# vpulab/GNN-CCA

Hardware: AMD Instinct MI355X
Metric: processed edges/sec (L=4 MPN steps), 256-node dense graph (higher is better)
Workload: dtype f32; 1 GPU; 1 x dense256 per GPU per step (N=256, E=65280), feat 2048, L=4, 3 cls steps, fp32, fp32 state, eval; mode=eager: MOTMPNet.forward, one call per step (auto: fastest one-at-a-time form), frames_in_flight=1, edge_state=fp32, edge_state_storage=f32, encoder_products=6, encoder_unsplit=False, outputs_finite=True, launcher=single process, ranks_seen=1

## Files before the change

gnn-cca_amd/csrc/internal.h:

```cpp
#pragma once
#include <stddef.h>
#include <stdint.h>

#include "gnncca_mpn.h"

namespace gnncca {

extern thread_local int g_last_hip_error;

const char* diag_env(const char* name);
int diag_env_int(const char* name, int fallback, int lo, int hi);

constexpr uint32_t kBlobMagic = 0x4D504E36u;
constexpr int kH = 32;
constexpr int kEF = 6;
constexpr int kProjOut = 48;
constexpr int kPdStride = 8;
constexpr int kPsQStride = 40;
constexpr int kMaxCls = 8;
constexpr int kMaxEdgeIn = 16;

enum Family : uint32_t {
    kFamilyNone = 0,
    kFamilyMfma32x6 = 1,
// ... 88 lines not shown
    auto take = [&at](auto*& field, int64_t count) { field = reinterpret_cast<decltype(+field)>(at), at += sizeof(*field) * (size_t)count; };
    StagingImage s;
    take(s.xw, n), take(s.yw, n), take(s.max_dist, g), take(s.ids, n), take(s.person, n), take(s.cam, n), take(s.graph_of, n);
    take(s.graph_ptr, g + 1), take(s.src_order, n), take(s.edge_ptr, n + 1), take(s.edge_ptr_g, g + 1);
    s.bytes = at - reinterpret_cast<uintptr_t>(base);
    return s;
}
inline size_t staging_image_bytes(int64_t n, int64_t g) { return n < 0 || g < 0 ? 0 : staging_image(nullptr, n, g).bytes; }

int build_edges_zeroing(const gnncca_frames* fr, const float* reid, int32_t reid_dim, int64_t n_nodes, int64_t n_edges, int32_t mode, bool capped,
                        int32_t top_k, int32_t rank_by, int32_t max_deg, int64_t* edge_index_out, float* edge_attr_out, float* edge_labels_out,
                        int32_t* zero_ptr, int64_t zero_n, gnncca_stream_t stream);

int build_edges_radius_zeroing(const gnncca_frames* fr, const float* reid, int32_t reid_dim, int64_t n_nodes, int64_t n_edges, int32_t mode,
                               double radius, int32_t unit, int64_t* edge_index_out, float* edge_attr_out, float* edge_labels_out,
                               int32_t* zero_ptr, int64_t zero_n, gnncca_stream_t stream);

Family classify(const gnncca_mpn_dims* d);
bool blob_header(const gnncca_mpn_dims* d, BlobHeader* out);
bool dims_valid(const gnncca_mpn_dims* d);
int mlp_param_count(const gnncca_mlp& m);

struct Workspace {
    size_t flags, blockflags, seg_ptr, col32, perm, cursor, h0, act, partial, pd[2], psq[2], e, e0, rng, total;
    int ksplit;
    int64_t e_stride;
    int ell_S;
};
int ell_stride(const gnncca_mpn_dims* d, int64_t n, int64_t e);
int enc_lds_ksplit(int64_t n_nodes, int K);
Workspace carve(const gnncca_mpn_dims* d, int64_t n, int64_t e);

enum EncForm : int {
    kEncPlanGemm = 0,
    kEncSlices,
    kEncD128,
    kEncR32Bf16,
    kEncR32F16,
    kEncLdsBf16,
    kEncLdsF16,
};
enum EncPlanPlace : int {
    kPlanNone = 0,
    kPlanRides,
    kPlanBefore,
    kPlanAfter,
};
// ... 34 lines not shown
    int kslice;
    int nst;
    int vec_ok;
};
struct EncRoute {
    int n_gemm;
    EncGemmRoute gemm[GNNCCA_MAX_LAYERS];
    bool split3, fused;
    int x_nt, force_arm;
    int plan_place, plan_span, plan_wgs;
    int tail, tail_npw, tail_vec;
    size_t tail_lds;
};
EncRoute encoder_route(const EncRouteIn& in, const EncTuning& t);

enum StepFamily : int {
    kStepGeneral = 0,
    kStepFast,
    kStepPipe,
};
#ifndef GNNCCA_NPW2_CLS
#define GNNCCA_NPW2_CLS 0
#endif
constexpr bool step_variant_exists(int family, bool FIRST, bool CLS, bool MSG, bool PDL, bool EB, int NT, bool RNG, int NPW, bool CIN) {
    if (family == kStepGeneral) return true;
    if (NT < 0 || NT > 2 || (NT != 0 && PDL)) return false;
    if (family == kStepFast) return !RNG && NPW == 1 && !CIN;
    if (CIN) return !FIRST && !PDL && !EB && !RNG && (MSG ? !CLS && (NPW == 1 || NPW == 2) : CLS && NPW == 1);
    if (RNG) return NT == 0 && NPW == 1;
    if (NPW == 2) return MSG && !PDL && (!CLS || GNNCCA_NPW2_CLS);
    return NPW == 1;
}
inline bool step_pipe_fits(long long N, long long E, long long e_stride, unsigned long long ws_bytes) {
    const long long lim = 1ll << 31;
    return 6 * e_stride * 4 <= lim && E * 16 <= lim && N * 32 <= lim && ws_bytes <= (unsigned long long)lim - 4096;
}
struct StepTuning {
    int msg_f32_max_n = 512;
    int fill_waves = 4096, fill_waves_long = 16384;
    int long_chunks = 32;
    int npw_min_n = 16384;
    int npw_min_n_first = 16384;
    int pd_lds_min = 0x7FFFFFFF, pd_lds_max = 1024;
    double nt_store_bytes = 150e6;
    double nt_load_bytes = 256e6;
    int force_wps = 0;
    int force_npw = 0;
    int force_nt = -1;
};
const StepTuning& step_tuning();
struct StepRouteIn {
    const gnncca_mpn_dims* d;
    const BlobHeader* hdr;
    const Workspace* ws;
    int N, E;
    uint32_t options;
    bool dropping;
    bool traced, trace_h_steps;
    bool attr_aligned;
};
struct StepPlan {
    int launches;
    int family;
    bool RE, MX;
    int N, hin;
    int msg_f32, attr_vec, wps, npw_first, npw_later, pd_lds, e_bf16;
    int nt;
    bool ranges;
    int ell_S;
    bool defer;
    bool trace_h_steps;
    int first_cls, L, cls_layers;
};
struct StepLaunch {
    int family;
    bool RE, MX, FIRST, CLS, MSG, PDL, EB;
    int NT;
    bool RNG;
    int NPW;
    bool CIN;
    unsigned blocks;
    size_t lds;
    int first, update, store_e, npw, cls_layers, cls_no, stamp_slot;
    int slot_out, slot_in;
    int buf_in, buf_out;
};
StepPlan step_plan(const StepRouteIn& in, const StepTuning& t);
StepLaunch step_launch(const StepPlan& p, int step);

struct BwdWorkspace {
    size_t gh0_acc, ge0_acc;
    size_t deg, Q;
    size_t hmax;
    size_t dP_all;
    size_t Hb[2], Gb[2], a1, gz1;
    size_t part;
    size_t bn_sums, bn_red;
    size_t total;
};
inline BwdWorkspace carve_backward(const gnncca_mpn_dims* d, int64_t n, int64_t e) {
    BwdWorkspace w;
    size_t off = 0;
    auto take = [&](size_t bytes) { size_t o = off; off += (bytes + 255) / 256 * 256; return o; };
    const size_t N = (size_t)(n > 0 ? n : 0), E = (size_t)(e > 0 ? e : 0), F1 = (size_t)d->enc_node.layers[0].out_dim;
    const size_t L = (size_t)(d->num_enc_steps > 1 ? d->num_enc_steps : 1);
    w.gh0_acc = take(N * kH * 4), w.ge0_acc = take(E * kEF * 4), w.deg = take(N * 4), w.Q = take(N * kH * 4);
    w.hmax = take(2 * N * kH * 4), w.dP_all = take(L * N * 44 * 4);
    for (int i = 0; i < 2; ++i) w.Hb[i] = take(N * kH * 4);
// ... 48 lines not shown
```

gnn-cca_amd/csrc/mpn_forward.hip:

```cpp
#include "forward_diag.cuh"
#include "wave_reduce.cuh"
#include "plan.cuh"
#include "encoder.cuh"
#include "enc_rows32.cuh"
#include "msg_bf16.cuh"
#include "step_general.cuh"
#include "step_fast.cuh"
#include "step_pipe.cuh"
#include "enc_f16.cuh"
#include "enc_f16_slices.cuh"
#include "generic_fused.cuh"
#include "generic.cuh"
#include "with_flag.h"

using namespace gnncca;

extern "C" {

#ifdef GNNCCA_STAMPS
__attribute__((visibility("default"))) int gnncca_debug_set_stamps(void* dev_buf) {
    unsigned long long* p = static_cast<unsigned long long*>(dev_buf);
    HIP_TRY(hipMemcpyToSymbol(HIP_SYMBOL(g_stamps), &p, sizeof(p)));
    return GNNCCA_OK;
}
// ... 5 lines not shown
    if (!workspace || !flags_out) return GNNCCA_ERR_INVALID_ARG;
    hipStream_t st = static_cast<hipStream_t>(stream);
    HIP_TRY(hipMemcpyAsync(flags_out, workspace, sizeof(uint32_t), hipMemcpyDeviceToHost, st));
    HIP_TRY(hipStreamSynchronize(st));
    return GNNCCA_OK;
}

int gnncca_read_graph_flags2(const void* workspace, uint32_t flags_out[2], gnncca_stream_t stream) {
    if (!workspace || !flags_out) return GNNCCA_ERR_INVALID_ARG;
    hipStream_t st = static_cast<hipStream_t>(stream);
    HIP_TRY(hipMemcpyAsync(flags_out, workspace, 2 * sizeof(uint32_t), hipMemcpyDeviceToHost, st));
    HIP_TRY(hipStreamSynchronize(st));
    return GNNCCA_OK;
}

}

static_assert(kEncSliceMaxK == kF16SlMaxKs, "encoder_route() sizes the slices of enc_f16_slices.cuh");

struct FwdBuffers {
    char* base;
    unsigned *flags, *blockflags;
    int *seg_ptr, *col32, *perm, *cursor;
    float *h0, *act, *part, *pd[2], *psq[2], *e, *e0;
};
static FwdBuffers carve_pointers(void* workspace, const Workspace& ws) {
    char* base = static_cast<char*>(workspace);
    auto f = [base](size_t off) { return reinterpret_cast<float*>(base + off); };
    auto i = [base](size_t off) { return reinterpret_cast<int*>(base + off); };
    auto u = [base](size_t off) { return reinterpret_cast<unsigned*>(base + off); };
    return FwdBuffers{base, u(ws.flags), u(ws.blockflags), i(ws.seg_ptr), i(ws.col32), i(ws.perm), i(ws.cursor), f(ws.h0), f(ws.act), f(ws.partial),
                      {f(ws.pd[0]), f(ws.pd[1])}, {f(ws.psq[0]), f(ws.psq[1])}, f(ws.e), f(ws.e0)};
}

template <class P>
static void fill_plan_finish(P& p, const FwdBuffers& b, const int64_t* edge_index, int E) {
    p.ei = reinterpret_cast<const long long*>(edge_index);
    p.seg_ptr = b.seg_ptr, p.col32 = b.col32, p.perm = b.perm, p.cursor = b.cursor, p.flags = b.flags, p.blockflags = b.blockflags;
    p.E = E;
}

static int enc_gemm_attributes() {
    static thread_local int attr_dev = -1;
    int dev = 0;
    HIP_TRY(hipGetDevice(&dev));
    if (attr_dev == dev) return GNNCCA_OK;
    HIP_TRY(hipFuncSetAttribute(reinterpret_cast<const void*>(enc_gemm_f16_fused_kernel), hipFuncAttributeMaxDynamicSharedMemorySize, (int)kF16LdsBytes));
    HIP_TRY(hipFuncSetAttribute(reinterpret_cast<const void*>(enc_gemm_f16_split_kernel), hipFuncAttributeMaxDynamicSharedMemorySize, (int)kF16LdsBytes));
    HIP_TRY(hipFuncSetAttribute(reinterpret_cast<const void*>(enc_gemm_f16_rows32_kernel), hipFuncAttributeMaxDynamicSharedMemorySize, (int)kF16R32LdsBytes));
    const void* fns[4] = {reinterpret_cast<const void*>(enc_gemm_split_lds_kernel<false, false>),
                          reinterpret_cast<const void*>(enc_gemm_split_lds_kernel<true, false>),
                          reinterpret_cast<const void*>(enc_gemm_split_lds_kernel<false, true>),
                          reinterpret_cast<const void*>(enc_gemm_split_lds_kernel<true, true>)};
    for (const void* fn : fns) HIP_TRY(hipFuncSetAttribute(fn, hipFuncAttributeMaxDynamicSharedMemorySize, (int)kLdsGemmBytes));
    attr_dev = dev;
// ... 174 lines not shown
    sp.hin = plan.hin;
    sp.msg_f32 = plan.msg_f32;
    sp.attr_vec = plan.attr_vec;
    sp.wps = plan.wps;
    sp.npw = plan.npw_later;
    sp.pd_lds = plan.pd_lds;
    sp.e_bf16 = plan.e_bf16;
    sp.ell_S = plan.ell_S;
    sp.nt_store = plan.nt >= 1, sp.nt_load = plan.nt >= 2;
    sp.rng = plan.ranges ? reinterpret_cast<int*>(b.base + ws.rng) : nullptr;
    sp.ws_base = b.base;
    sp.ws_bytes = ws.total;
    sp.so_e = (unsigned)ws.e, sp.so_col = (unsigned)ws.col32, sp.so_perm = (unsigned)ws.perm;
    sp.drop = drop;
    return sp;
}

static hipError_t launch_step_variant(const StepLaunch& l, const StepParams& sp, hipStream_t st) {
    const dim3 grid(l.blocks), block(256);
    bool launched = false;
    auto with_nt = [&](auto&& f) {
        l.NT == 2 ? f(std::integral_constant<int, 2>{}) : l.NT == 1 ? f(std::integral_constant<int, 1>{}) : f(std::integral_constant<int, 0>{});
    };
    if (l.family == kStepGeneral) {
        with_flag(l.RE, [&](auto RE) { with_flag(l.MSG, [&](auto MSG) { with_flag(l.MX, [&](auto MX) {
            GNNCCA_LAUNCH((mpn_step_kernel<RE(), MSG(), MX()>), grid, block, l.lds, st, sp);
            launched = true;
        }); }); });
    } else {
        with_flag(l.FIRST, [&](auto FIRST) { with_flag(l.CLS, [&](auto CLS) { with_flag(l.MSG, [&](auto MSG) { with_flag(l.PDL, [&](auto PDL) {
        with_nt([&](auto NT) { with_flag(l.EB, [&](auto EB) {
            if (l.family == kStepFast) {
                if constexpr (step_variant_exists(kStepFast, FIRST(), CLS(), MSG(), PDL(), EB(), NT(), false, 1, false)) {
                    GNNCCA_LAUNCH((mpn_step_fast_kernel<FIRST(), CLS(), MSG(), PDL(), EB(), NT()>), grid, block, l.lds, st, sp);
                    launched = true;
                }
                return;
            }
            with_flag(l.RNG, [&](auto RNG) { with_flag(l.NPW == 2, [&](auto TWO) { with_flag(l.CIN, [&](auto CIN) {
                constexpr int NPW = TWO() ? 2 : 1;
                if constexpr (step_variant_exists(kStepPipe, FIRST(), CLS(), MSG(), PDL(), EB(), NT(), RNG(), NPW, CIN())) {
                    GNNCCA_LAUNCH((mpn_step_pipe_kernel<FIRST(), CLS(), MSG(), PDL(), EB(), NT(), RNG(), NPW, CIN()>), grid, block, l.lds, st, sp);
                    launched = true;
                }
            }); }); });
        }); });
        }); }); }); });
    }
    return launched ? hipGetLastError() : hipErrorInvalidValue;
}

static int forward_impl(const gnncca_mpn_dims* d, const void* packed_dev, const float* x, const int64_t* edge_index,
                        const float* edge_attr, int64_t n_nodes, int64_t n_edges, void* workspace, size_t workspace_bytes,
                        float* logits_out, const gnncca_trace* trace, gnncca_stream_t stream, Profiler* prof,
                        uint32_t options, const gnncca_dropout* dropout = nullptr) {
    if (!dims_valid(d) || n_nodes < 0 || n_edges < 0) return GNNCCA_ERR_INVALID_ARG;
    const Family fam = classify(d);
    if (fam == kFamilyNone) return GNNCCA_ERR_UNSUPPORTED;
    if (n_nodes >= (1ll << 31) - 64 || n_edges >= (1ll << 31) - 64) return GNNCCA_ERR_UNSUPPORTED;
    if (n_nodes == 0) return n_edges == 0 ? GNNCCA_OK : GNNCCA_ERR_INVALID_ARG;
    if (!packed_dev || !x || !workspace) return GNNCCA_ERR_INVALID_ARG;
// ... 35 lines not shown

    StepParams sp = step_setup(plan, d, hdr, ws, b, blob, edge_attr, N, E, drop);
    for (int i = 0; i < plan.launches; ++i) {
        const int step = plan.L == 0 ? 0 : i + 1;
        const StepLaunch l = step_launch(plan, step);
        sp.first = l.first;
        sp.update = l.update;
        sp.store_e = l.store_e;
        sp.npw = l.npw;
        sp.step_no = step;
        sp.cls_no = l.cls_no;
        sp.stamp_slot = l.stamp_slot;
        sp.cls_layers = l.cls_layers;
        sp.logits = l.slot_out >= 0 ? logits_out + (size_t)l.slot_out * E : nullptr;
        sp.logits_in = l.slot_in >= 0 ? logits_out + (size_t)l.slot_in * E : nullptr;
        sp.pd_in = l.buf_in >= 0 ? b.pd[l.buf_in] : nullptr;
        sp.so_pd = l.buf_in >= 0 ? (unsigned)ws.pd[l.buf_in] : 0u;
        sp.psq_in = l.buf_in >= 0 ? b.psq[l.buf_in] : nullptr;
        sp.pd_out = l.buf_out >= 0 ? b.pd[l.buf_out] : nullptr;
        sp.psq_out = l.buf_out >= 0 ? b.psq[l.buf_out] : nullptr;
        sp.trace_e_enc = (trace && l.first) ? trace->e_enc : nullptr;
        sp.trace_e = (trace && trace->e_steps && l.update) ? trace->e_steps + (size_t)(step - 1) * E * kEF : nullptr;
        sp.trace_h = (plan.trace_h_steps && l.update) ? trace->h_steps + (size_t)(step - 1) * N * kH : nullptr;
        HIP_TRY(launch_step_variant(l, sp, st));
        PROF_MARK(l.MSG ? GNNCCA_K_STEP : GNNCCA_K_STEP_LAST);
    }
    return GNNCCA_OK;
}

extern "C" {

int gnncca_mpn_forward(const gnncca_mpn_dims* d, const void* packed_dev, const float* x, const int64_t* edge_index,
                       const float* edge_attr, int64_t n_nodes, int64_t n_edges, void* workspace, size_t workspace_bytes,
                       float* logits_out, const gnncca_trace* trace, gnncca_stream_t stream) {
    return forward_impl(d, packed_dev, x, edge_index, edge_attr, n_nodes, n_edges, workspace, workspace_bytes, logits_out,
                        trace, stream, nullptr, 0u);
}

int gnncca_mpn_forward_ex(const gnncca_mpn_dims* d, const void* packed_dev, const float* x, const int64_t* edge_index,
                          const float* edge_attr, int64_t n_nodes, int64_t n_edges, void* workspace, size_t workspace_bytes,
                          float* logits_out, const gnncca_trace* trace, uint32_t options, gnncca_stream_t stream) {
    return forward_impl(d, packed_dev, x, edge_index, edge_attr, n_nodes, n_edges, workspace, workspace_bytes, logits_out,
                        trace, stream, nullptr, options);
}

int gnncca_mpn_forward_train(const gnncca_mpn_dims* d, const void* packed_dev, const float* x, const int64_t* edge_index,
// ... 25 lines not shown
```

gnn-cca_amd/csrc/pack.cpp:

```cpp
#include <algorithm>
#include <cmath>
#include <cstdio>
#include <cstdlib>
#include <cstring>
#include <vector>

#include "internal.h"

namespace gnncca {

thread_local int g_last_hip_error = 0;

static inline size_t align_up(size_t v, size_t a) { return (v + a - 1) / a * a; }

int mlp_param_count(const gnncca_mlp& m) {
    int n = 0;
    for (int i = 0; i < m.n_layers; ++i) n += 2 + (m.layers[i].has_bn ? 4 : 0);
    return n;
}

static bool mlp_chain_ok(const gnncca_mlp& m, int in_dim, int out_dim) {
    if (m.n_layers < 0 || m.n_layers > GNNCCA_MAX_LAYERS) return false;
    if (m.n_layers == 0) return in_dim == out_dim;
    int cur = in_dim;
// ... 596 lines not shown
    w.row32o = take(E * 4);
    w.col32o = take(E * 4);
    for (int i = 0; i < 3; ++i) w.node[i] = take(N * (size_t)nw * 4);
    w.h0 = take(N * (size_t)d->node_dim * 4);
    for (int i = 0; i < 4; ++i) w.edge[i] = take(E * (size_t)ew * 4);
    w.e0 = take(E * (size_t)d->edge_dim * 4);
    const int ks = gen_enc0_ksplit(d, n);
    w.partial = take(ks > 0 ? (size_t)ks * N * (size_t)d->enc_node.layers[0].out_dim * 4 : 0);
    {
        const size_t o1e = d->edge_mlp.n_layers > 0 ? (size_t)d->edge_mlp.layers[0].out_dim : 0;
        const size_t o1n = d->node_mlp.n_layers > 0 ? (size_t)d->node_mlp.layers[0].out_dim : 0;
        for (int i = 0; i < 2; ++i) w.tab[i] = take(N * (2 * o1e + o1n) * 4);
    }
    w.total = off;
    return w;
}

static const char* const kDiagSwitches[] = {
    "GNNCCA_DIAG", "GNNCCA_LIB", "GNNCCA_STAMPS",
    "GNNCCA_GEMM_SPLIT_MIN", "GNNCCA_GEMM_LDS_MIN", "GNNCCA_GEMM_R32F_MIN", "GNNCCA_GEMM_R32F_MAX",
    "GNNCCA_GEMM_SLICES_MIN", "GNNCCA_GEMM_SLICES_MAX", "GNNCCA_GEMM_SLICES_NKS", "GNNCCA_GEMM_SLICES_WGS",
    "GNNCCA_GEMM_BF16", "GNNCCA_GEMM_F16_ARM", "GNNCCA_GEMM_F16_XNT", "GNNCCA_TAIL_MFMA_MIN",
    "GNNCCA_WPS", "GNNCCA_NPW", "GNNCCA_NPW_MIN_N", "GNNCCA_NPW_MIN_N_FIRST",
    "GNNCCA_STEP_NT", "GNNCCA_PD_LDS_MIN", "GNNCCA_PD_LDS_MAX", "GNNCCA_NO_PAD",
    "GNNCCA_GEN_UNFUSED", "GNNCCA_COLNORM_NOLDS", "GNNCCA_POOL_CHUNK", "GNNCCA_POOL_SPIN_US"};

extern "C" char** environ;

const char* diag_env(const char* name) {
    static const bool on = [] {
        const char* v = std::getenv("GNNCCA_DIAG");
        const bool open = v != nullptr && v[0] == '1' && v[1] == '\0';
        if (open && environ) {
            for (char** e = environ; *e; ++e) {
                if (std::strncmp(*e, "GNNCCA_", 7) != 0) continue;
                const char* eq = std::strchr(*e, '=');
                const size_t len = eq ? (size_t)(eq - *e) : std::strlen(*e);
                bool known = false;
                for (const char* k : kDiagSwitches) known = known || (std::strlen(k) == len && std::strncmp(k, *e, len) == 0);
                if (!known) {
                    std::fprintf(stderr, "[gnncca] GNNCCA_DIAG=1: '%.*s' is not a switch of this build and is ignored; recognised:", (int)len, *e);
                    for (const char* k : kDiagSwitches) std::fprintf(stderr, " %s", k);
                    std::fprintf(stderr, "\n");
                }
            }
        }
        return open;
// ... 51 lines not shown
    int ks = 1;
    while (ks < 32 && row_tiles * (size_t)ks < 512 && k0 / (ks * 2) >= 64) ks *= 2;
    if (N >= 1024)
        while (ks < 8 && ((N + 127) / 128) * (size_t)ks < 512 && k0 / (ks * 2) >= 64) ks *= 2;
    if (N >= 4096) ks = std::max(ks, enc_lds_ksplit((int64_t)N, k0));
    w.ksplit = ks;
    size_t fmax = 0;
    for (int i = 0; i < d->enc_node.n_layers; ++i)
        fmax = fmax > (size_t)d->enc_node.layers[i].out_dim ? fmax : (size_t)d->enc_node.layers[i].out_dim;
    w.flags = take(256);
    w.blockflags = take((E / 256 + 2) * 4);
    w.seg_ptr = take((N + 1) * 4);
    w.col32 = take(E * 4);
    w.perm = take(E * 4);
    w.cursor = take((N + 1) * 4);
    w.h0 = take(N * kH * 4);
    w.act = take(d->enc_node.n_layers >= 3 ? 2 * N * fmax * 4 : 0);
    w.partial = take((size_t)ks * N * fmax * 4);
    for (int i = 0; i < 2; ++i) w.pd[i] = take(N * kPdStride * 4);
    for (int i = 0; i < 2; ++i) w.psq[i] = take(N * kPsQStride * 4);
    w.e = take((size_t)kEF * w.e_stride * 4);
    w.e0 = take(d->reattach_edges ? (size_t)kEF * w.e_stride * 4 : 0);
    w.rng = take(N * 16);
    w.total = off;
    return w;
}

}

extern "C" size_t gnncca_workspace_bytes(const gnncca_mpn_dims* d, int64_t n_nodes, int64_t n_edges) {
    const Family fam = classify(d);
    if (fam == kFamilyNone || n_nodes < 0 || n_edges < 0) return 0;
    if (fam == kFamilyGeneric) return carve_generic(d, n_nodes, n_edges).total;
    return carve(d, n_nodes, n_edges).total;
}
```

gnn-cca_amd/csrc/step_fast.cuh:

```cuda
#pragma once
namespace gnncca {

__device__ __forceinline__ float relu_bits(float x) { return __int_as_float(max(__float_as_int(x), 0)); }

#ifdef GNNCCA_FAST_WAVES
#define GNNCCA_FAST_ATTR __attribute__((amdgpu_waves_per_eu(GNNCCA_FAST_WAVES, GNNCCA_FAST_WAVES)))
#else
#define GNNCCA_FAST_ATTR __attribute__((amdgpu_waves_per_eu(MSG ? 4 : 1)))
#endif
template <bool FIRST, bool CLS, bool MSG, bool PD_LDS, bool EBF16, int NT>
__global__ __launch_bounds__(256) GNNCCA_FAST_ATTR void mpn_step_fast_kernel(const StepParams p) {
    extern __shared__ __attribute__((aligned(16))) float smem[];
    float* s_proj = smem;
    float* s_part = s_proj + (MSG ? kH * kProjOut : 0);
    int* s_rng = reinterpret_cast<int*>(s_part + 4 * kH);
    float* s_pd = s_part + 4 * kH + 16;
    const int tid = threadIdx.x, lane = tid & 63;
    const int wave = __builtin_amdgcn_readfirstlane(tid >> 6);
    const float* __restrict__ blob = p.blob;
    constexpr bool DERIVE = FIRST && MSG;
    typedef const float __attribute__((address_space(4))) cfloat;
    cfloat* cw = (cfloat*)(unsigned long long)(blob + p.off_fast);

    GNNCCA_STAMP(p.stamp_slot, 0);
    const int ktouch = touch_kernargs(sizeof(StepParams));
    const unsigned gflags = p.flags[0];
    const unsigned rbad = p.flags[1];
    const int wps = p.wps;
    const int wl = wps >> 1;
    const int node = (int)(blockIdx.x << (2 - wl)) + (wave >> wl);
    const int sub = wave & (wps - 1);
    const bool active = node < p.N;
    const int nclamp = active ? node : 0;
    int seg_s = p.seg_ptr[nclamp];
    int seg_t = p.seg_ptr[nclamp + 1];
    const bool use_range = !FIRST && p.rng != nullptr && rbad == 0u;
    int rs1 = 0, rl1 = 0, rd2 = 0;
    if (!FIRST && p.rng != nullptr) {
        typedef int i32x4 __attribute__((ext_vector_type(4)));
        const i32x4 r = reinterpret_cast<const i32x4*>(p.rng)[nclamp];
        rs1 = r[0], rl1 = r[1], rd2 = r[2];
    }
    asm volatile("" ::"s"(gflags), "s"(rbad), "s"(seg_s), "s"(seg_t), "s"(rs1), "s"(rl1), "s"(rd2), "s"(ktouch));
    const int nmax = p.N - 1;
    const int half = lane >> 5, ch = lane & 31;
    const float* __restrict__ psq = p.psq_in + (size_t)nclamp * kPsQStride;
    float psrc[kEF];
    float cinit = 0.f;
    float bw[3] = {0.f, 0.f, 0.f};
    f32x4 stage_proj[2];
    f32x4 stage_pd[8];
    float projb_l = 0.f;
    const int pd_n4 = p.N * (kPdStride / 4);
    auto request_node_operands = [&]() {
#pragma unroll
        for (int f = 0; f < kEF; ++f) psrc[f] = psq[f];
        if (MSG) {
            cinit = psq[8 + ch];
            projb_l = blob[p.off_projb + min(lane, kProjOut - 1)];
#pragma unroll
            for (int s = 0; s < 3; ++s) bw[s] = blob[p.off_wneb + s * 64 + lane];
            const f32x4* __restrict__ g4 = reinterpret_cast<const f32x4*>(blob + p.off_projwT);
            stage_proj[0] = g4[tid];
            stage_proj[1] = g4[min(tid + 256, kH * kProjOut / 4 - 1)];
        }
        if (PD_LDS) {
            const f32x4* __restrict__ g4 = reinterpret_cast<const f32x4*>(p.pd_in);
#pragma unroll
            for (int i = 0; i < 8; ++i) stage_pd[i] = g4[min(tid + i * 256, pd_n4 - 1)];
        }
    };
    if (gflags & GNNCCA_GRAPH_BAD_INDEX) {
        if (CLS)
            for (size_t k = (size_t)blockIdx.x * 256 + tid; k < (size_t)p.E; k += (size_t)gridDim.x * 256)
                p.logits[k] = __builtin_nanf("");
        return;
    }
    const bool unsorted = (gflags & GNNCCA_GRAPH_UNSORTED) != 0;
    if (!active) seg_s = seg_t = 0;
    const long long eoff = (p.ell_S > 0 && !(gflags & (GNNCCA_GRAPH_UNSORTED | GNNCCA_GRAPH_IRREGULAR)))
                               ? (long long)nclamp * p.ell_S - seg_s : 0ll;

    constexpr bool nt_store = NT >= 1, nt_load = NT >= 2;
    f32x16 acc;
#pragma unroll
    for (int i = 0; i < 16; ++i) acc[i] = 0.f;
    const int last = seg_t - 1;

    struct Chunk {
        float raw[kEF];
        float pd[kEF];
        int ko, j;
        int jp;
    };
    auto load_index = [&](int base, Chunk& c) {
        const int kk = max(min(base + lane, last), 0);
        c.ko = unsorted ? p.perm[kk] : kk;
        int cj = 0;
        if (!FIRST) {
            const int q = kk - seg_s;
            cj = max(min(q + (q < rl1 ? rs1 : rd2), nmax), 0);
            asm volatile("" : "+v"(cj));
        }
        if (!use_range) {
            cj = p.col32[kk];
            if (DERIVE) c.jp = p.col32[max(kk - 1, 0)];
        }
        c.j = cj;
    };
    int d_nb = 0, d_first = 0x7FFFFFFF, d_start2 = 0, d_start1 = 0;
    auto derive = [&](int base, const Chunk& c) {
        const int k = base + lane;
        const bool brk = k < seg_t && k > seg_s && c.j != c.jp + 1;
        const unsigned long long m = __ballot(brk);
        if (m != 0ull) {
            if (d_nb == 0) {
                const int l = __ffsll((long long)m) - 1;
                d_first = base + l - seg_s;
                d_start2 = __builtin_amdgcn_readlane(c.j, l);
            }
            d_nb += __popcll(m);
        }
        if (base == seg_s) d_start1 = __builtin_amdgcn_readfirstlane(c.j);
    };
    auto load_state = [&](int base, Chunk& c) {
        const int kk = max(min(base + lane, last), 0);
        if (FIRST) {
            const f32x4* __restrict__ ap = reinterpret_cast<const f32x4*>(p.edge_attr + (size_t)c.ko * 4);
            const f32x4 a = nt_store ? __builtin_nontemporal_load(ap) : *ap;
            c.raw[0] = a[0], c.raw[1] = a[1], c.raw[2] = a[2], c.raw[3] = a[3], c.raw[4] = 0.f, c.raw[5] = 0.f;
        } else if (EBF16) {
            const unsigned* __restrict__ e2 = reinterpret_cast<const unsigned*>(p.e);
#pragma unroll
            for (int f = 0; f < kEF / 2; ++f) {
                const unsigned w = nt_load ? __builtin_nontemporal_load(e2 + (size_t)f * p.e_stride + kk + eoff)
                                           : e2[(size_t)f * p.e_stride + kk + eoff];
                c.raw[2 * f] = __uint_as_float(w << 16);
                c.raw[2 * f + 1] = __uint_as_float(w & 0xFFFF0000u);
            }
        } else {
            if (nt_load) {
#pragma unroll
                for (int f = 0; f < kEF; ++f) c.raw[f] = __builtin_nontemporal_load(p.e + (size_t)f * p.e_stride + kk + eoff);
            } else {
#pragma unroll
                for (int f = 0; f < kEF; ++f) c.raw[f] = p.e[(size_t)f * p.e_stride + kk + eoff];
            }
        }
    };
    auto load_target = [&](Chunk& c) {
        f32x4 a;
        f32x2 b2;
        if (PD_LDS) {
            a = *reinterpret_cast<const f32x4*>(s_pd + c.j * kPdStride);
            b2 = *reinterpret_cast<const f32x2*>(s_pd + c.j * kPdStride + 4);
        } else {
            const float* __restrict__ pdj = p.pd_in + (size_t)c.j * kPdStride;
            a = *reinterpret_cast<const f32x4*>(pdj);
            b2 = *reinterpret_cast<const f32x2*>(pdj + 4);
        }
        c.pd[0] = a[0], c.pd[1] = a[1], c.pd[2] = a[2], c.pd[3] = a[3], c.pd[4] = b2[0], c.pd[5] = b2[1];
    };
    auto compute_chunk = [&](int base, const Chunk& c) {
        const int k = base + lane;
        const bool valid = k < seg_t;
        float ein[kEF];
        if (FIRST) {
#pragma unroll
            for (int h = 0; h < kEF / 2; ++h) {
                f32x2 s = {cw[kFcEncB + 2 * h], cw[kFcEncB + 2 * h + 1]};
#pragma unroll
                for (int q = 0; q < 4; ++q) {
                    const f32x2 w = {cw[kFcEncW + q * kEF + 2 * h], cw[kFcEncW + q * kEF + 2 * h + 1]};
                    s = __builtin_elementwise_fma(w, f32x2{c.raw[q], c.raw[q]}, s);
                }
                ein[2 * h] = fmaxf(s[0], 0.f), ein[2 * h + 1] = fmaxf(s[1], 0.f);
            }
        } else {
#pragma unroll
            for (int f = 0; f < kEF; ++f) ein[f] = c.raw[f];
        }
        float en[kEF];
        f32x2 s2[kEF / 2];
#pragma unroll
        for (int h = 0; h < kEF / 2; ++h) s2[h] = f32x2{psrc[2 * h], psrc[2 * h + 1]} + f32x2{c.pd[2 * h], c.pd[2 * h + 1]};
#pragma unroll
        for (int g = 0; g < kEF; ++g) {
            const f32x2 x = {ein[g], ein[g]};
#pragma unroll
            for (int h = 0; h < kEF / 2; ++h) {
                const f32x2 w = {cw[kFcWee + g * kEF + 2 * h], cw[kFcWee + g * kEF + 2 * h + 1]};
                s2[h] = __builtin_elementwise_fma(w, x, s2[h]);
            }
        }
#pragma unroll
        for (int h = 0; h < kEF / 2; ++h) en[2 * h] = fmaxf(s2[h][0], 0.f), en[2 * h + 1] = fmaxf(s2[h][1], 0.f);
        if (p.store_e && valid) {
            if (EBF16) {
                unsigned* __restrict__ e2 = reinterpret_cast<unsigned*>(p.e);
#pragma unroll
                for (int f = 0; f < kEF / 2; ++f) {
                    typedef __bf16 bf16x2_t __attribute__((ext_vector_type(2)));
                    bf16x2_t pk;
                    pk[0] = (__bf16)en[2 * f];
                    pk[1] = (__bf16)en[2 * f + 1];
                    if (nt_store)
                        __builtin_nontemporal_store(__builtin_bit_cast(unsigned, pk), e2 + (size_t)f * p.e_stride + k + eoff);
                    else
                        e2[(size_t)f * p.e_stride + k + eoff] = __builtin_bit_cast(unsigned, pk);
                }
            } else {
#pragma unroll
                for (int f = 0; f < kEF; ++f) {
                    if (nt_store)
                        __builtin_nontemporal_store(en[f], p.e + (size_t)f * p.e_stride + k + eoff);
                    else
                        p.e[(size_t)f * p.e_stride + k + eoff] = en[f];
                }
            }
        }
// ... 44 lines not shown
            }
        }
    };

    const int stride = 64 * wps;
    int base = seg_s + 64 * sub;
    Chunk c0, c1;
    load_index(base, c0);
    load_index(base + stride, c1);
    __builtin_amdgcn_sched_barrier(0);
    request_node_operands();
    __builtin_amdgcn_sched_barrier(0);
    load_state(base, c0);
    load_state(base + stride, c1);
    __builtin_amdgcn_sched_barrier(0);
    if (!PD_LDS) {
        load_target(c0);
        load_target(c1);
    }
    if (MSG) {
        f32x4* l4 = reinterpret_cast<f32x4*>(s_proj);
        l4[tid] = stage_proj[0];
        if (tid + 256 < kH * kProjOut / 4) l4[tid + 256] = stage_proj[1];
    }
    if (PD_LDS) {
        f32x4* l4 = reinterpret_cast<f32x4*>(s_pd);
#pragma unroll
        for (int i = 0; i < 8; ++i)
            if (tid + i * 256 < pd_n4) l4[tid + i * 256] = stage_pd[i];
    }
    GNNCCA_STAMP(p.stamp_slot, 1);
    if (PD_LDS || (MSG && (wps == 1 || (p.diag & 8)))) __syncthreads();
    GNNCCA_STAMP(p.stamp_slot, 2);
    auto round_body = [&](int rb, Chunk& a, Chunk& b, bool requested = false) {
        if (!requested) {
            load_target(a);
            load_target(b);
        }
        if (DERIVE && p.rng != nullptr) {
            derive(rb, a);
            if (rb + stride < seg_t) derive(rb + stride, b);
        }
        GNNCCA_STAMP(p.stamp_slot, 3);
        compute_chunk(rb, a);
        if (rb + stride < seg_t) compute_chunk(rb + stride, b);
        GNNCCA_STAMP(p.stamp_slot, 4);
// ... 78 lines not shown
```

gnn-cca_amd/csrc/step_general.cuh:

```cuda
#pragma once
namespace gnncca {

struct StepParams {
    const float* blob;
    const int* seg_ptr;
    const int* col32;
    const int* perm;
    unsigned* flags;
    const float* edge_attr;
    float* e;
    float* e0;
    const float* pd_in;
    const float* psq_in;
    float* pd_out;
    float* psq_out;
    const float* h0;
    float* trace_h;
    float* trace_e;
    float* trace_e_enc;
    float* logits;
    float* logits_in;
    long long e_stride;
    int off_wee, off_wneb, off_projwT, off_projb, off_encw, off_encb, off_cw1, off_cb1, off_cw2, off_cb2;
    int off_fast;
    int off_wnebf;
    int cls_layers, cls_hidden;
    int N, E, edge_in, attr_vec, first, update, agg, reatt_n, wps, store_e, hin, pd_lds, stamp_slot, e_bf16;
    int ell_S;
    int nt_store, nt_load;
    DropCfg drop;
    int step_no, cls_no;
    int msg_f32;
    int* rng;
    const void* ws_base;
    unsigned long long ws_bytes;
    unsigned so_e, so_col, so_perm, so_pd;
    int npw;
    int diag;
};

template <bool REATT_E, bool MSG, bool AGG_MAX>
__global__ __launch_bounds__(256) void mpn_step_kernel(const StepParams p) {
// ... 259 lines not shown
```

gnn-cca_amd/csrc/step_route.cpp:

```cpp
#include <algorithm>

#include "internal.h"

namespace gnncca {

const StepTuning& step_tuning() {
    static const StepTuning tuning = [] {
        StepTuning t;
        const int inf = 0x7FFFFFFF;
        t.force_wps = diag_env_int("GNNCCA_WPS", t.force_wps, 1, 4);
        t.force_npw = diag_env_int("GNNCCA_NPW", t.force_npw, 1, 2);
        t.npw_min_n = diag_env_int("GNNCCA_NPW_MIN_N", t.npw_min_n, 0, inf);
        t.npw_min_n_first = diag_env_int("GNNCCA_NPW_MIN_N_FIRST", t.npw_min_n_first, 0, inf);
        t.pd_lds_max = diag_env_int("GNNCCA_PD_LDS_MAX", t.pd_lds_max, 0, 1024);
        t.pd_lds_min = diag_env_int("GNNCCA_PD_LDS_MIN", t.pd_lds_min, 0, inf);
        t.force_nt = diag_env_int("GNNCCA_STEP_NT", t.force_nt, -1, 2);
        return t;
    }();
    return tuning;
}

StepPlan step_plan(const StepRouteIn& in, const StepTuning& t) {
    const gnncca_mpn_dims* d = in.d;
    const BlobHeader& hdr = *in.hdr;
    const Workspace& ws = *in.ws;
    const int N = in.N, E = in.E, L = d->num_enc_steps;
    StepPlan p{};
    p.launches = E <= 0 ? 0 : (L == 0 ? 1 : L);
    p.N = N, p.L = L;
    p.first_cls = L - d->num_class_steps + 1;
    p.cls_layers = hdr.cls_layers;
    p.hin = (d->reattach_nodes ? 2 : 1) * kH;
    p.RE = d->reattach_edges != 0, p.MX = d->agg == GNNCCA_AGG_MAX;
    p.trace_h_steps = in.traced && in.trace_h_steps;
    p.msg_f32 = (N <= t.msg_f32_max_n || !step_pipe_fits(N, E, ws.e_stride, ws.total)) ? 1 : 0;
    p.attr_vec = d->edge_in == 4 && in.attr_aligned;
    const bool special = hdr.fast_consts != 0 && p.attr_vec && !in.traced && !p.MX;
    p.family = (L == 0 || !special) ? kStepGeneral : (p.msg_f32 ? kStepFast : kStepPipe);
    p.ell_S = (ws.ell_S > 0 && special && E > 0) ? ws.ell_S : 0;

    const long long avg_deg = (E + (long long)N - 1) / N;
    const int chunks = (int)((avg_deg + 63) / 64);
    const int by_chunks = chunks >= 4 ? 4 : (chunks >= 2 ? 2 : 1);
    const long long want = (chunks >= t.long_chunks ? t.fill_waves_long : t.fill_waves) / (long long)N;
    int wps = by_chunks;
    while (wps > 1 && wps > want) wps >>= 1;
    if ((in.options & GNNCCA_OPT_ENC_UNSPLIT) != 0 && N >= 4096) wps = 1;
    if (t.force_wps == 1 || t.force_wps == 2 || t.force_wps == 4) wps = std::min(t.force_wps, by_chunks);
    p.wps = wps;
    p.npw_later = (wps == 1 && chunks <= 2 && (t.force_npw == 2 || (t.force_npw == 0 && N >= t.npw_min_n))) ? 2 : 1;
    p.npw_first = (p.npw_later == 2 && (t.force_npw == 2 || N >= t.npw_min_n_first)) ? 2 : 1;
    p.ranges = L >= 2 && (in.options & GNNCCA_OPT_COLUMN_RANGES) != 0;
    p.pd_lds = (N >= t.pd_lds_min && N <= t.pd_lds_max) && L > 0;
    p.e_bf16 = (in.options & GNNCCA_OPT_EDGE_STATE_BF16) != 0;
    const double state_bytes = (double)(p.e_bf16 ? kEF / 2 : kEF) * (double)ws.e_stride * 4.0;
    p.nt = state_bytes > t.nt_load_bytes ? 2 : (state_bytes > t.nt_store_bytes ? 1 : 0);
    if (t.force_nt >= 0) p.nt = t.force_nt;
    p.defer = p.family == kStepPipe && !p.e_bf16 && !p.pd_lds && !p.ranges && p.first_cls < L && !in.dropping && p.npw_later == 2;
    return p;
}

StepLaunch step_launch(const StepPlan& p, int step) {
    const int L = p.L;
    StepLaunch l{};
    l.family = p.family, l.RE = p.RE, l.MX = p.MX, l.NPW = 1;
    l.first = step <= 1, l.update = step >= 1, l.store_e = step >= 1 && step < L;
    l.npw = step == 1 ? p.npw_first : p.npw_later;
    l.stamp_slot = step >= 1 ? 2 + std::min(step - 1, 5) : 0;
    l.MSG = step >= 1 && (step < L || p.trace_h_steps);
    l.buf_in = step >= 1 ? (step - 1) & 1 : -1;
    l.buf_out = l.store_e ? step & 1 : -1;
    const bool classifies = step == 0 || step >= p.first_cls;
    l.slot_out = l.slot_in = -1;
    if (p.defer) {
        if (step == L) l.slot_out = L - p.first_cls;
        if (step - 1 >= p.first_cls) l.slot_in = step - 1 - p.first_cls;
    } else if (classifies) {
        l.slot_out = l.cls_no = std::max(0, step - std::max(p.first_cls, 1));
    }
    l.cls_layers = l.slot_out >= 0 ? p.cls_layers : 0;
    l.CLS = l.cls_layers != 0;

    const int npg = 4 / p.wps;
    l.blocks = (unsigned)((p.N + npg - 1) / npg);
    if (p.family == kStepGeneral) {
        l.lds = ((l.MSG ? (size_t)p.hin * kProjOut : 0) + 4 * kH + (p.pd_lds ? (size_t)p.N * kPdStride : 0)) * sizeof(float);
        return l;
    }
    const bool two = l.npw == 2 && p.wps == 1;
    if (l.slot_in >= 0) {
        l.FIRST = false, l.CIN = true, l.NT = p.nt;
        l.NPW = l.MSG && two ? 2 : 1;
    } else {
        l.FIRST = l.first, l.PDL = p.pd_lds, l.EB = p.e_bf16;
        l.NT = l.PDL ? 0 : p.nt;
        if (p.family == kStepPipe) {
            l.RNG = p.ranges && l.NT == 0 && (!l.FIRST || l.MSG);
            l.NPW = two && !p.ranges && step_variant_exists(kStepPipe, l.FIRST, l.CLS, l.MSG, l.PDL, l.EB, l.NT, false, 2, false) ? 2 : 1;
        }
    }
    if (l.NPW == 2) l.blocks = (unsigned)((p.N + 7) / 8);
    const size_t pd_rows = !l.PDL ? 0 : (size_t)p.N + (p.family == kStepPipe ? 1 : 0);
    l.lds = ((l.MSG ? (size_t)kH * kProjOut : 0) + 4 * kH + 16 + pd_rows * kPdStride) * sizeof(float);
    return l;
// ... 4 lines not shown
```

Baseline: 2.194 billion edges/s.

## Elide edge-state stores and recompute them in the next MPN step

Adds an RC template mode to the fast step kernel. Selected message steps skip writing the fp32 edge state. The following step rebuilds it by reapplying the previous edge update from the prior node projections, which are saved to a side buffer when the double-buffered pd/psq would be overwritten. This trades edge-state store and load traffic for extra per-edge FMAs and an extra pd gather. It also drops the waves-per-EU hint for recompute variants, which risks register pressure and occupancy changes. Trace pointers are unioned with the new pointers.

```diff
diff --git a/gnn-cca_amd/csrc/internal.h b/gnn-cca_amd/csrc/internal.h
--- a/gnn-cca_amd/csrc/internal.h
+++ b/gnn-cca_amd/csrc/internal.h
@@ -134,7 +134,7 @@
 int mlp_param_count(const gnncca_mlp& m);
 
 struct Workspace {
-    size_t flags, blockflags, seg_ptr, col32, perm, cursor, h0, act, partial, pd[2], psq[2], e, e0, rng, total;
+    size_t flags, blockflags, seg_ptr, col32, perm, cursor, h0, act, partial, pd[2], psq[2], e, e0, rng, side, total;
     int ksplit;
     int64_t e_stride;
     int ell_S;
@@ -215,9 +215,11 @@
 #ifndef GNNCCA_NPW2_CLS
 #define GNNCCA_NPW2_CLS 0
 #endif
-constexpr bool step_variant_exists(int family, bool FIRST, bool CLS, bool MSG, bool PDL, bool EB, int NT, bool RNG, int NPW, bool CIN) {
-    if (family == kStepGeneral) return true;
+constexpr bool step_variant_exists(int family, bool FIRST, bool CLS, bool MSG, bool PDL, bool EB, int NT, bool RNG, int NPW, bool CIN, int RC = 0) {
+    if (family == kStepGeneral) return RC == 0;
     if (NT < 0 || NT > 2 || (NT != 0 && PDL)) return false;
+    if (RC != 0)
+        return family == kStepFast && RC >= 1 && RC <= 3 && !PDL && !EB && NT == 0 && !RNG && NPW == 1 && !CIN && (RC == 1 ? MSG : !FIRST && (CLS || MSG));
     if (family == kStepFast) return !RNG && NPW == 1 && !CIN;
     if (CIN) return !FIRST && !PDL && !EB && !RNG && (MSG ? !CLS && (NPW == 1 || NPW == 2) : CLS && NPW == 1);
     if (RNG) return NT == 0 && NPW == 1;
@@ -240,6 +242,7 @@
     int force_wps = 0;
     int force_npw = 0;
     int force_nt = -1;
+    int recompute = 2;
 };
 const StepTuning& step_tuning();
 struct StepRouteIn {
@@ -262,6 +265,7 @@
     bool ranges;
     int ell_S;
     bool defer;
+    int recompute;
     bool trace_h_steps;
     int first_cls, L, cls_layers;
 };
@@ -277,6 +281,12 @@
     int first, update, store_e, npw, cls_layers, cls_no, stamp_slot;
     int slot_out, slot_in;
     int buf_in, buf_out;
+    bool elided;
+    bool recomputes;
+    bool from_attr;
+    bool side_out;
+    bool side_in;
+    int RC;
 };
 StepPlan step_plan(const StepRouteIn& in, const StepTuning& t);
 StepLaunch step_launch(const StepPlan& p, int step);
diff --git a/gnn-cca_amd/csrc/mpn_forward.hip b/gnn-cca_amd/csrc/mpn_forward.hip
--- a/gnn-cca_amd/csrc/mpn_forward.hip
+++ b/gnn-cca_amd/csrc/mpn_forward.hip
@@ -51,7 +51,7 @@
     char* base;
     unsigned *flags, *blockflags;
     int *seg_ptr, *col32, *perm, *cursor;
-    float *h0, *act, *part, *pd[2], *psq[2], *e, *e0;
+    float *h0, *act, *part, *pd[2], *psq[2], *e, *e0, *side;
 };
 static FwdBuffers carve_pointers(void* workspace, const Workspace& ws) {
     char* base = static_cast<char*>(workspace);
@@ -59,7 +59,7 @@
     auto i = [base](size_t off) { return reinterpret_cast<int*>(base + off); };
     auto u = [base](size_t off) { return reinterpret_cast<unsigned*>(base + off); };
     return FwdBuffers{base, u(ws.flags), u(ws.blockflags), i(ws.seg_ptr), i(ws.col32), i(ws.perm), i(ws.cursor), f(ws.h0), f(ws.act), f(ws.partial),
-                      {f(ws.pd[0]), f(ws.pd[1])}, {f(ws.psq[0]), f(ws.psq[1])}, f(ws.e), f(ws.e0)};
+                      {f(ws.pd[0]), f(ws.pd[1])}, {f(ws.psq[0]), f(ws.psq[1])}, f(ws.e), f(ws.e0), f(ws.side)};
 }
 
 template <class P>
@@ -280,6 +280,12 @@
     auto with_nt = [&](auto&& f) {
         l.NT == 2 ? f(std::integral_constant<int, 2>{}) : l.NT == 1 ? f(std::integral_constant<int, 1>{}) : f(std::integral_constant<int, 0>{});
     };
+    auto with_rc = [&](auto&& f) {
+        l.RC == 3   ? f(std::integral_constant<int, 3>{})
+        : l.RC == 2 ? f(std::integral_constant<int, 2>{})
+        : l.RC == 1 ? f(std::integral_constant<int, 1>{})
+                    : f(std::integral_constant<int, 0>{});
+    };
     if (l.family == kStepGeneral) {
         with_flag(l.RE, [&](auto RE) { with_flag(l.MSG, [&](auto MSG) { with_flag(l.MX, [&](auto MX) {
             GNNCCA_LAUNCH((mpn_step_kernel<RE(), MSG(), MX()>), grid, block, l.lds, st, sp);
@@ -289,12 +295,15 @@
         with_flag(l.FIRST, [&](auto FIRST) { with_flag(l.CLS, [&](auto CLS) { with_flag(l.MSG, [&](auto MSG) { with_flag(l.PDL, [&](auto PDL) {
         with_nt([&](auto NT) { with_flag(l.EB, [&](auto EB) {
             if (l.family == kStepFast) {
-                if constexpr (step_variant_exists(kStepFast, FIRST(), CLS(), MSG(), PDL(), EB(), NT(), false, 1, false)) {
-                    GNNCCA_LAUNCH((mpn_step_fast_kernel<FIRST(), CLS(), MSG(), PDL(), EB(), NT()>), grid, block, l.lds, st, sp);
-                    launched = true;
-                }
+                with_rc([&](auto RC) {
+                    if constexpr (step_variant_exists(kStepFast, FIRST(), CLS(), MSG(), PDL(), EB(), NT(), false, 1, false, RC())) {
+                        GNNCCA_LAUNCH((mpn_step_fast_kernel<FIRST(), CLS(), MSG(), PDL(), EB(), NT(), RC()>), grid, block, l.lds, st, sp);
+                        launched = true;
+                    }
+                });
                 return;
             }
+            if (l.RC != 0) return;
             with_flag(l.RNG, [&](auto RNG) { with_flag(l.NPW == 2, [&](auto TWO) { with_flag(l.CIN, [&](auto CIN) {
                 constexpr int NPW = TWO() ? 2 : 1;
                 if constexpr (step_variant_exists(kStepPipe, FIRST(), CLS(), MSG(), PDL(), EB(), NT(), RNG(), NPW, CIN())) {
@@ -376,6 +385,11 @@
         sp.trace_e_enc = (trace && l.first) ? trace->e_enc : nullptr;
         sp.trace_e = (trace && trace->e_steps && l.update) ? trace->e_steps + (size_t)(step - 1) * E * kEF : nullptr;
         sp.trace_h = (plan.trace_h_steps && l.update) ? trace->h_steps + (size_t)(step - 1) * N * kH : nullptr;
+        if (l.RC != 0) {
+            sp.pd_prev = !l.recomputes ? nullptr : (l.side_in ? b.side : b.pd[l.buf_in ^ 1]);
+            sp.psq_prev = !l.recomputes ? nullptr : (l.side_in ? b.side + (size_t)N * kPdStride : b.psq[l.buf_in ^ 1]);
+            sp.side_out = l.side_out ? b.side : nullptr;
+        }
         HIP_TRY(launch_step_variant(l, sp, st));
         PROF_MARK(l.MSG ? GNNCCA_K_STEP : GNNCCA_K_STEP_LAST);
     }
diff --git a/gnn-cca_amd/csrc/pack.cpp b/gnn-cca_amd/csrc/pack.cpp
--- a/gnn-cca_amd/csrc/pack.cpp
+++ b/gnn-cca_amd/csrc/pack.cpp
@@ -642,7 +642,7 @@
     "GNNCCA_GEMM_SLICES_MIN", "GNNCCA_GEMM_SLICES_MAX", "GNNCCA_GEMM_SLICES_NKS", "GNNCCA_GEMM_SLICES_WGS",
     "GNNCCA_GEMM_BF16", "GNNCCA_GEMM_F16_ARM", "GNNCCA_GEMM_F16_XNT", "GNNCCA_TAIL_MFMA_MIN",
     "GNNCCA_WPS", "GNNCCA_NPW", "GNNCCA_NPW_MIN_N", "GNNCCA_NPW_MIN_N_FIRST",
-    "GNNCCA_STEP_NT", "GNNCCA_PD_LDS_MIN", "GNNCCA_PD_LDS_MAX", "GNNCCA_NO_PAD",
+    "GNNCCA_STEP_NT", "GNNCCA_STEP_RECOMPUTE", "GNNCCA_PD_LDS_MIN", "GNNCCA_PD_LDS_MAX", "GNNCCA_NO_PAD",
     "GNNCCA_GEN_UNFUSED", "GNNCCA_COLNORM_NOLDS", "GNNCCA_POOL_CHUNK", "GNNCCA_POOL_SPIN_US"};
 
 extern "C" char** environ;
@@ -740,6 +740,7 @@
     w.e = take((size_t)kEF * w.e_stride * 4);
     w.e0 = take(d->reattach_edges ? (size_t)kEF * w.e_stride * 4 : 0);
     w.rng = take(N * 16);
+    w.side = take(N * (size_t)(kPdStride + kPsQStride) * 4);
     w.total = off;
     return w;
 }
diff --git a/gnn-cca_amd/csrc/step_fast.cuh b/gnn-cca_amd/csrc/step_fast.cuh
--- a/gnn-cca_amd/csrc/step_fast.cuh
+++ b/gnn-cca_amd/csrc/step_fast.cuh
@@ -6,10 +6,15 @@
 #ifdef GNNCCA_FAST_WAVES
 #define GNNCCA_FAST_ATTR __attribute__((amdgpu_waves_per_eu(GNNCCA_FAST_WAVES, GNNCCA_FAST_WAVES)))
 #else
-#define GNNCCA_FAST_ATTR __attribute__((amdgpu_waves_per_eu(MSG ? 4 : 1)))
+#define GNNCCA_FAST_ATTR __attribute__((amdgpu_waves_per_eu(MSG && RC < 2 ? 4 : 1)))
 #endif
-template <bool FIRST, bool CLS, bool MSG, bool PD_LDS, bool EBF16, int NT>
+template <bool FIRST, bool CLS, bool MSG, bool PD_LDS, bool EBF16, int NT, int RC = 0>
 __global__ __launch_bounds__(256) GNNCCA_FAST_ATTR void mpn_step_fast_kernel(const StepParams p) {
+    static_assert(RC == 0 || (!PD_LDS && !EBF16 && NT == 0), "recomputed edge state: fp32 state, no LDS table, default cache policy");
+    static_assert(RC != 1 || MSG, "only a message step's store is elided");
+    static_assert(RC < 2 || !FIRST, "step 1 has nothing to recompute");
+    constexpr bool ELIDE = RC == 1, RECOMP = RC >= 2;
+    constexpr bool ATTR = FIRST || RC == 3;
     extern __shared__ __attribute__((aligned(16))) float smem[];
     float* s_proj = smem;
     float* s_part = s_proj + (MSG ? kH * kProjOut : 0);
@@ -46,6 +51,8 @@
     const int half = lane >> 5, ch = lane & 31;
     const float* __restrict__ psq = p.psq_in + (size_t)nclamp * kPsQStride;
     float psrc[kEF];
+    float psrc0[kEF];
+    float side_v = 0.f;
     float cinit = 0.f;
     float bw[3] = {0.f, 0.f, 0.f};
     f32x4 stage_proj[2];
@@ -55,6 +62,16 @@
     auto request_node_operands = [&]() {
 #pragma unroll
         for (int f = 0; f < kEF; ++f) psrc[f] = psq[f];
+        if (RECOMP) {
+            const float* __restrict__ psq0 = p.psq_prev + (size_t)nclamp * kPsQStride;
+#pragma unroll
+            for (int f = 0; f < kEF; ++f) psrc0[f] = psq0[f];
+        }
+        if (ELIDE) {
+            const float* __restrict__ row = lane < kPdStride ? p.pd_in + (size_t)nclamp * kPdStride + lane
+                                                             : psq + (min(lane, kProjOut - 1) - kPdStride);
+            side_v = *row;
+        }
         if (MSG) {
             cinit = psq[8 + ch];
             projb_l = blob[p.off_projb + min(lane, kProjOut - 1)];
@@ -90,6 +107,7 @@
     struct Chunk {
         float raw[kEF];
         float pd[kEF];
+        float pd0[kEF];
         int ko, j;
         int jp;
     };
@@ -125,7 +143,7 @@
     };
     auto load_state = [&](int base, Chunk& c) {
         const int kk = max(min(base + lane, last), 0);
-        if (FIRST) {
+        if (ATTR) {
             const f32x4* __restrict__ ap = reinterpret_cast<const f32x4*>(p.edge_attr + (size_t)c.ko * 4);
             const f32x4 a = nt_store ? __builtin_nontemporal_load(ap) : *ap;
             c.raw[0] = a[0], c.raw[1] = a[1], c.raw[2] = a[2], c.raw[3] = a[3], c.raw[4] = 0.f, c.raw[5] = 0.f;
@@ -160,12 +178,34 @@
             b2 = *reinterpret_cast<const f32x2*>(pdj + 4);
         }
         c.pd[0] = a[0], c.pd[1] = a[1], c.pd[2] = a[2], c.pd[3] = a[3], c.pd[4] = b2[0], c.pd[5] = b2[1];
+        if (RECOMP) {
+            const float* __restrict__ pd0j = p.pd_prev + (size_t)c.j * kPdStride;
+            const f32x4 a0 = *reinterpret_cast<const f32x4*>(pd0j);
+            const f32x2 b0 = *reinterpret_cast<const f32x2*>(pd0j + 4);
+            c.pd0[0] = a0[0], c.pd0[1] = a0[1], c.pd0[2] = a0[2], c.pd0[3] = a0[3], c.pd0[4] = b0[0], c.pd0[5] = b0[1];
+        }
+    };
+    auto edge_update = [&](const float* ein, const float* ps, const float* pd, float* en) {
+        f32x2 s2[kEF / 2];
+#pragma unroll
+        for (int h = 0; h < kEF / 2; ++h) s2[h] = f32x2{ps[2 * h], ps[2 * h + 1]} + f32x2{pd[2 * h], pd[2 * h + 1]};
+#pragma unroll
+        for (int g = 0; g < kEF; ++g) {
+            const f32x2 x = {ein[g], ein[g]};
+#pragma unroll
+            for (int h = 0; h < kEF / 2; ++h) {
+                const f32x2 w = {cw[kFcWee + g * kEF + 2 * h], cw[kFcWee + g * kEF + 2 * h + 1]};
+                s2[h] = __builtin_elementwise_fma(w, x, s2[h]);
+            }
+        }
+#pragma unroll
+        for (int h = 0; h < kEF / 2; ++h) en[2 * h] = fmaxf(s2[h][0], 0.f), en[2 * h + 1] = fmaxf(s2[h][1], 0.f);
     };
     auto compute_chunk = [&](int base, const Chunk& c) {
         const int k = base + lane;
         const bool valid = k < seg_t;
         float ein[kEF];
-        if (FIRST) {
+        if (ATTR) {
 #pragma unroll
             for (int h = 0; h < kEF / 2; ++h) {
                 f32x2 s = {cw[kFcEncB + 2 * h], cw[kFcEncB + 2 * h + 1]};
@@ -181,21 +221,14 @@
             for (int f = 0; f < kEF; ++f) ein[f] = c.raw[f];
         }
         float en[kEF];
-        f32x2 s2[kEF / 2];
-#pragma unroll
-        for (int h = 0; h < kEF / 2; ++h) s2[h] = f32x2{psrc[2 * h], psrc[2 * h + 1]} + f32x2{c.pd[2 * h], c.pd[2 * h + 1]};
-#pragma unroll
-        for (int g = 0; g < kEF; ++g) {
-            const f32x2 x = {ein[g], ein[g]};
-#pragma unroll
-            for (int h = 0; h < kEF / 2; ++h) {
-                const f32x2 w = {cw[kFcWee + g * kEF + 2 * h], cw[kFcWee + g * kEF + 2 * h + 1]};
-                s2[h] = __builtin_elementwise_fma(w, x, s2[h]);
-            }
-        }
-#pragma unroll
-        for (int h = 0; h < kEF / 2; ++h) en[2 * h] = fmaxf(s2[h][0], 0.f), en[2 * h + 1] = fmaxf(s2[h][1], 0.f);
-        if (p.store_e && valid) {
+        if (RECOMP) {
+            float emid[kEF];
+            edge_update(ein, psrc0, c.pd0, emid);
+            edge_update(emid, psrc, c.pd, en);
+        } else {
+            edge_update(ein, psrc, c.pd, en);
+        }
+        if (!ELIDE && p.store_e && valid) {
             if (EBF16) {
                 unsigned* __restrict__ e2 = reinterpret_cast<unsigned*>(p.e);
 #pragma unroll
@@ -286,6 +319,13 @@
         f32x4* l4 = reinterpret_cast<f32x4*>(s_proj);
         l4[tid] = stage_proj[0];
         if (tid + 256 < kH * kProjOut / 4) l4[tid + 256] = stage_proj[1];
+    }
+    if (ELIDE) {
+        if (p.side_out != nullptr && active && sub == 0 && lane < kProjOut) {
+            float* row = lane < kPdStride ? p.side_out + (size_t)node * kPdStride + lane
+                                          : p.side_out + (size_t)p.N * kPdStride + (size_t)node * kPsQStride + (lane - kPdStride);
+            *row = side_v;
+        }
     }
     if (PD_LDS) {
         f32x4* l4 = reinterpret_cast<f32x4*>(s_pd);
diff --git a/gnn-cca_amd/csrc/step_general.cuh b/gnn-cca_amd/csrc/step_general.cuh
--- a/gnn-cca_amd/csrc/step_general.cuh
+++ b/gnn-cca_amd/csrc/step_general.cuh
@@ -15,9 +15,18 @@
     float* pd_out;
     float* psq_out;
     const float* h0;
-    float* trace_h;
-    float* trace_e;
-    float* trace_e_enc;
+    union {
+        float* trace_h;
+        const float* pd_prev;
+    };
+    union {
+        float* trace_e;
+        const float* psq_prev;
+    };
+    union {
+        float* trace_e_enc;
+        float* side_out;
+    };
     float* logits;
     float* logits_in;
     long long e_stride;
diff --git a/gnn-cca_amd/csrc/step_route.cpp b/gnn-cca_amd/csrc/step_route.cpp
--- a/gnn-cca_amd/csrc/step_route.cpp
+++ b/gnn-cca_amd/csrc/step_route.cpp
@@ -15,6 +15,7 @@
         t.pd_lds_max = diag_env_int("GNNCCA_PD_LDS_MAX", t.pd_lds_max, 0, 1024);
         t.pd_lds_min = diag_env_int("GNNCCA_PD_LDS_MIN", t.pd_lds_min, 0, inf);
         t.force_nt = diag_env_int("GNNCCA_STEP_NT", t.force_nt, -1, 2);
+        t.recompute = diag_env_int("GNNCCA_STEP_RECOMPUTE", t.recompute, 0, 2);
         return t;
     }();
     return tuning;
@@ -57,6 +58,7 @@
     p.nt = state_bytes > t.nt_load_bytes ? 2 : (state_bytes > t.nt_store_bytes ? 1 : 0);
     if (t.force_nt >= 0) p.nt = t.force_nt;
     p.defer = p.family == kStepPipe && !p.e_bf16 && !p.pd_lds && !p.ranges && p.first_cls < L && !in.dropping && p.npw_later == 2;
+    p.recompute = (p.family == kStepFast && N <= t.msg_f32_max_n && L >= 2 && !p.e_bf16 && !p.pd_lds && p.nt == 0) ? t.recompute : 0;
     return p;
 }
 
@@ -80,6 +82,17 @@
     }
     l.cls_layers = l.slot_out >= 0 ? p.cls_layers : 0;
     l.CLS = l.cls_layers != 0;
+    auto elides = [&](int s) {
+        bool e = false;
+        for (int k = 1; k <= s; ++k) e = k < L && !e && (p.recompute == 2 ? (k & 1) != 0 || k == L - 1 : p.recompute == 1 && k == L - 1);
+        return e;
+    };
+    l.elided = step >= 1 && elides(step);
+    l.recomputes = step >= 2 && elides(step - 1);
+    l.from_attr = l.recomputes && step == 2;
+    l.side_out = l.elided && step + 1 < L;
+    l.side_in = l.recomputes && step < L;
+    l.RC = l.elided ? 1 : (l.recomputes ? (l.from_attr ? 3 : 2) : 0);
 
     const int npg = 4 / p.wps;
     l.blocks = (unsigned)((p.N + npg - 1) / npg);
```

Measured after the change: 2.046 billion edges/s. -6.7%, worse.
